# bioinformatics-ua/polus

Measured on AMD Instinct MI355X. Metric: train samples/sec BioBERT-base NER seq256, higher is better.
Workload: dtype bf16

## Files before the change

### polus_amd/csrc/attention.hip

```cpp
#include "common.h"

namespace {

constexpr int D = 64;
constexpr int BLK = 64;
constexpr float MASK_NEG = -10000.0f;
constexpr float LOG2E = 1.4426950408889634f, LN2 = 0.6931471805599453f;

template <typename T> struct TileCfg;
template <> struct TileCfg<bf16_t> { static constexpr int RS = 160, EPC = 8, LOG_CPR = 3, NLOAD = 2; };
template <> struct TileCfg<float> { static constexpr int RS = 288, EPC = 4, LOG_CPR = 4, NLOAD = 4; };

template <typename T, int NT = 256>
__device__ __forceinline__ void tile_load(unsigned char* tile, const T* __restrict__ base, long ld, int row0,
                                          int nrows, int col0, int tid) {
    constexpr int LOG = TileCfg<T>::LOG_CPR;
#pragma unroll
    for (int k = 0; k < TileCfg<T>::NLOAD; ++k) {
        int c = tid + NT * k;
        int r = c >> LOG, ch = c & ((1 << LOG) - 1);
        uint4 v = make_uint4(0, 0, 0, 0);
        if (row0 + r < nrows)
            v = *reinterpret_cast<const uint4*>(base + (long)(row0 + r) * ld + col0 + ch * TileCfg<T>::EPC);
        *reinterpret_cast<uint4*>(tile + r * TileCfg<T>::RS + ch * 16) = v;
// ... 37 lines not shown

__device__ __forceinline__ void frag_from_acc(Frag<bf16_t>& f, const f32x4& t0, const f32x4& t1) {
    f.v[0] = (bf16_t)t0[0]; f.v[1] = (bf16_t)t0[1]; f.v[2] = (bf16_t)t0[2]; f.v[3] = (bf16_t)t0[3];
    f.v[4] = (bf16_t)t1[0]; f.v[5] = (bf16_t)t1[1]; f.v[6] = (bf16_t)t1[2]; f.v[7] = (bf16_t)t1[3];
}
__device__ __forceinline__ void frag_from_acc(Frag<float>& f, const f32x4& t0, const f32x4& t1) {
    f.v[0] = t0[0]; f.v[1] = t0[1]; f.v[2] = t0[2]; f.v[3] = t0[3];
    f.v[4] = t1[0]; f.v[5] = t1[1]; f.v[6] = t1[2]; f.v[7] = t1[3];
}

__device__ __forceinline__ float col_max(float v) { v = fmaxf(v, __shfl_xor(v, 16, 64)); return fmaxf(v, __shfl_xor(v, 32, 64)); }
__device__ __forceinline__ float col_sum(float v) { v += __shfl_xor(v, 16, 64); return v + __shfl_xor(v, 32, 64); }

template <typename T>
__device__ __forceinline__ void store_acc_T(T* __restrict__ out, long ld, int row, int col0, const f32x4 (&o)[4],
                                            float mul, int g, bool valid) {
    if (!valid) return;
#pragma unroll
    for (int dt = 0; dt < 4; ++dt) {
        float v[4] = {o[dt][0] * mul, o[dt][1] * mul, o[dt][2] * mul, o[dt][3] * mul};
        store4<T>(out + (long)row * ld + col0 + dt * 16 + 4 * g, v);
    }
}

struct AttnArgs {
    const void* qkv; const int32_t* mask; void* ctx; float* lse;
    const void* dctx; const float* delta; void* dqkv;
    int B, S, A, H;
    float scale;
    unsigned drop_thresh, drop_seed;
    float drop_inv;
    const PolusDyn* dyn;
    int debug;
};

__device__ __forceinline__ float key_bias(const int32_t* mask, int b, int S, int key) {
    if (key >= S) return -INFINITY;
    if (!mask) return 0.0f;
    return (1.0f - (float)mask[(long)b * S + key]) * MASK_NEG;
}

template <typename T, int NW>
__global__ __launch_bounds__(64 * NW) void attn_fwd_kernel(AttnArgs p) {
    if (p.drop_thresh) p.drop_seed = polus_eff_seed(p.drop_seed, p.dyn);
    constexpr int QB = 16 * NW, NT = 64 * NW;
    extern __shared__ __attribute__((aligned(16))) unsigned char smem[];
    unsigned char* Kc = smem;
    unsigned char* Vc = smem + QB * TileCfg<T>::RS;
    float* kbc = reinterpret_cast<float*>(smem + 2 * QB * TileCfg<T>::RS);
    const int tid = threadIdx.x, lane = tid & 63, wid = tid >> 6, i = lane & 15, g = lane >> 4;
    const int q0 = blockIdx.x * QB, h = blockIdx.y, b = blockIdx.z;
    const int S = p.S, H = p.H;
    const long ld = 3L * H;
    const T* qkv = static_cast<const T*>(p.qkv) + (long)b * S * ld;
    const int q = q0 + wid * 16 + i;
    const bool qvalid = q < S;

    Frag<T> qf[2];
#pragma unroll
    for (int sub = 0; sub < 2; ++sub)
        frag_global<T>(qf[sub], qkv + (long)q * ld + h * D + sub * 32 + 8 * g, qvalid);

    const float scale2 = p.scale * LOG2E;
    float m = -1e30f, l = 0.f;
    f32x4 o[4];
#pragma unroll
    for (int dt = 0; dt < 4; ++dt) o[dt] = (f32x4){0.f, 0.f, 0.f, 0.f};
// ... 117 lines not shown

    auto issue_block = [&](int j) {
        unsigned char* st = ring + (j & 3) * FWD_STAGE;
#pragma unroll
        for (int e = 0; e < PPW; ++e) {
            const int piece = wid + e * NW;
            const int row = min(j * BLK + (piece & 7) * 8 + r8, S - 1);
            dma16(qkv + (long)row * ld + (piece < 8 ? H : 2 * H) + h * D + src_chunk, st + piece * 1024);
        }
    };
    const int nblk = (S + BLK - 1) / BLK;
    if (p.mask)
        for (int k0 = wid * 64; k0 < S; k0 += 64 * NW)
            dma4(p.mask + (long)b * S + min(k0 + lane, S - 1), reinterpret_cast<unsigned char*>(kbc) + k0 * 4);
    {
        unsigned char* qs = ring + 3 * FWD_STAGE;
#pragma unroll
        for (int e = 0; e < 2; ++e) {
            const int piece = wid + e * NW;
            dma16(qkv + (long)min(q0 + piece * 8 + r8, S - 1) * ld + h * D + src_chunk, qs + piece * 1024);
        }
    }
#pragma unroll
    for (int j = 0; j < 3; ++j) if (j < nblk) issue_block(j);
    wait_blocks_left<PPW>(min(nblk, 3));
    __builtin_amdgcn_s_barrier();
    Frag<T> qf[2];
    {
        const int row = wid * 16 + i;
#pragma unroll
        for (int sub = 0; sub < 2; ++sub)
            qf[sub].v = *reinterpret_cast<const bf16x8*>(ring + 3 * FWD_STAGE + row * 128 + (((sub * 4 + g) ^ (row & 7)) * 16));
    }
    for (int t = tid; t < nblk * BLK; t += NT) {
        float bias = 0.0f;
        if (p.mask) bias = (1.0f - (float)reinterpret_cast<const int*>(kbc)[t]) * MASK_NEG;
        kbc[t] = t < S ? bias * LOG2E : -INFINITY;
    }
    wait_lgkm();
    __builtin_amdgcn_s_barrier();
    if (nblk > 3) issue_block(3);
    int issued = min(nblk, 4);

    const float scale2 = p.scale * LOG2E;
    float m = -1e30f, l = 0.f;
    f32x4 o[4];
#pragma unroll
    for (int dt = 0; dt < 4; ++dt) o[dt] = (f32x4){0.f, 0.f, 0.f, 0.f};
    const int kx = i & 7;
    const int k_off0 = i * 128 + ((g ^ kx) * 16), k_off1 = i * 128 + (((4 + g) ^ kx) * 16);
    const int vrow = 4 * g + (i >> 2), vx = vrow & 7;
    const int v_base = vrow * 128 + (i & 1) * 8, v_c = (i & 3) >> 1;

    for (int j0 = 0; j0 < nblk; j0 += 2) {
        const bool two = j0 + 1 < nblk;
        f32x4 s[2][4];
#pragma unroll
        for (int jj = 0; jj < 2; ++jj) {
            if (jj == 0 || two) {
                wait_blocks_left<PPW>(issued - 1 - (j0 + jj));
                __builtin_amdgcn_s_barrier();
                const unsigned char* Kt = ring + ((j0 + jj) & 3) * FWD_STAGE;
#pragma unroll
                for (int kt = 0; kt < 4; ++kt) {
                    s[jj][kt] = (f32x4){0.f, 0.f, 0.f, 0.f};
                    Frag<T> a0, a1;
                    a0.v = *reinterpret_cast<const bf16x8*>(Kt + kt * 2048 + k_off0);
                    a1.v = *reinterpret_cast<const bf16x8*>(Kt + kt * 2048 + k_off1);
                    mma16(s[jj][kt], a0, qf[0]);
                    mma16(s[jj][kt], a1, qf[1]);
                }
            } else {
#pragma unroll
                for (int kt = 0; kt < 4; ++kt) s[jj][kt] = (f32x4){-INFINITY, -INFINITY, -INFINITY, -INFINITY};
            }
        }
        float mx = -INFINITY;
#pragma unroll
        for (int jj = 0; jj < 2; ++jj)
            if (jj == 0 || two) {
#pragma unroll
                for (int kt = 0; kt < 4; ++kt) {
                    const f32x4 kb = *reinterpret_cast<const f32x4*>(kbc + (j0 + jj) * BLK + kt * 16 + 4 * g);
#pragma unroll
                    for (int r = 0; r < 4; ++r) s[jj][kt][r] = fmaf(s[jj][kt][r], scale2, kb[r]);
                    mx = fmaxf(mx, fmaxf(fmaxf(s[jj][kt][0], s[jj][kt][1]), fmaxf(s[jj][kt][2], s[jj][kt][3])));
                }
            }
        mx = col_max2(mx);
        const float m_new = fmaxf(m, mx);
        const float alpha = __builtin_amdgcn_exp2f(m - m_new);
        m = m_new;
        float rs = 0.f;
        Frag<T> pf[2][2];
#pragma unroll
        for (int jj = 0; jj < 2; ++jj) {
#pragma unroll
            for (int kt = 0; kt < 4; ++kt)
#pragma unroll
                for (int r = 0; r < 4; ++r) { s[jj][kt][r] = __builtin_amdgcn_exp2f(s[jj][kt][r] - m_new); rs += s[jj][kt][r]; }
            if (p.drop_thresh) {
                const unsigned rowb = (((unsigned)b * p.A + h) * S + (unsigned)q) * S + (j0 + jj) * BLK + 4 * g;
#pragma unroll
                for (int kt = 0; kt < 4; ++kt) {
                    float t4[4] = {s[jj][kt][0], s[jj][kt][1], s[jj][kt][2], s[jj][kt][3]};
                    polus_dropout_run<4>(t4, p.drop_seed, rowb + kt * 16, p.drop_thresh, p.drop_inv, (S & 3) == 0);
                    s[jj][kt] = (f32x4){t4[0], t4[1], t4[2], t4[3]};
                }
            }
            frag_from_acc(pf[jj][0], s[jj][0], s[jj][1]);
            frag_from_acc(pf[jj][1], s[jj][2], s[jj][3]);
        }
        l = l * alpha + rs;
#pragma unroll
        for (int dt = 0; dt < 4; ++dt)
#pragma unroll
            for (int r = 0; r < 4; ++r) o[dt][r] *= alpha;
#pragma unroll
        for (int jj = 0; jj < 2; ++jj) {
            if (jj == 0 || two) {
                const unsigned char* Vt = ring + ((j0 + jj) & 3) * FWD_STAGE + BLK * 128 + v_base;
#pragma unroll
                for (int ks = 0; ks < 2; ++ks)
#pragma unroll
                    for (int dt = 0; dt < 4; ++dt) {
                        const unsigned char* vp = Vt + ks * 4096 + (((2 * dt + v_c) ^ vx) * 16);
                        const s16x4 lo = lds_tr16(vp), hi = lds_tr16(vp + 16 * 128);
                        typedef short s16x8 __attribute__((ext_vector_type(8)));
                        const s16x8 w = {lo[0], lo[1], lo[2], lo[3], hi[0], hi[1], hi[2], hi[3]};
                        Frag<T> va;
                        va.v = __builtin_bit_cast(bf16x8, w);
                        mma16(o[dt], va, pf[jj][ks]);
                    }
            }
        }
        if (j0 + 4 < nblk) {
            wait_lgkm();
            __builtin_amdgcn_s_barrier();
            issue_block(j0 + 4);
            ++issued;
            if (j0 + 5 < nblk) { issue_block(j0 + 5); ++issued; }
        }
    }
    l = col_sum2(l);
    const float inv_l = 1.0f / l;
    wait_lgkm();
    __builtin_amdgcn_s_barrier();
    unsigned char* ot = ring + wid * 2048;
#pragma unroll
    for (int dt = 0; dt < 4; ++dt) {
        float v[4] = {o[dt][0] * inv_l, o[dt][1] * inv_l, o[dt][2] * inv_l, o[dt][3] * inv_l};
        store4<T>(reinterpret_cast<T*>(ot + i * 128 + (((2 * dt + (g >> 1)) ^ (i & 7)) * 16) + (g & 1) * 8), v);
    }
    wait_lgkm();
    T* ctx = static_cast<T*>(p.ctx) + (long)b * S * H;
#pragma unroll
    for (int t = 0; t < 2; ++t) {
        const int row = 8 * t + r8, qq = q0 + wid * 16 + row;
        const uint4 v = *reinterpret_cast<const uint4*>(ot + row * 128 + (lane & 7) * 16);
        if (qq < S) *reinterpret_cast<uint4*>(ctx + (long)qq * H + h * D + (((lane & 7) ^ (row & 7)) * 8)) = v;
    }
    if (q < S && g == 0) p.lse[((long)b * p.A + h) * S + q] = m * LN2 + __logf(l);
}

template <typename T, int NW>
__global__ __launch_bounds__(64 * NW) void attn_bwd_dq_kernel(AttnArgs p) {
    if (p.drop_thresh) p.drop_seed = polus_eff_seed(p.drop_seed, p.dyn);
    constexpr int QB = 16 * NW, NT = 64 * NW;
// ... 343 lines not shown
__device__ __forceinline__ unsigned lds_off(const unsigned char* p) { return (unsigned)(unsigned long)(const lds_u8*)p; }
template <int ROW16>
__device__ __forceinline__ void tr_pair_asm(Frag<bf16_t>& f, unsigned addr) {
    v2i_t lo, hi;
    asm volatile("ds_read_b64_tr_b16 %0, %2\n\tds_read_b64_tr_b16 %1, %2 offset:%3" : "=&v"(lo), "=&v"(hi) : "v"(addr), "n"(ROW16));
    typedef int v4i_t __attribute__((ext_vector_type(4)));
    const v4i_t w = {lo[0], lo[1], hi[0], hi[1]};
    f.v = __builtin_bit_cast(bf16x8, w);
}
__device__ __forceinline__ void ds_read128_asm(Frag<bf16_t>& f, unsigned addr) {
    typedef int v4i_t __attribute__((ext_vector_type(4)));
    v4i_t w;
    asm volatile("ds_read_b128 %0, %1" : "=&v"(w) : "v"(addr));
    f.v = __builtin_bit_cast(bf16x8, w);
}
__device__ __forceinline__ uint2 ds_read64_asm(unsigned addr) {
    v2i_t w;
    asm volatile("ds_read_b64 %0, %1" : "=&v"(w) : "v"(addr));
    return make_uint2((unsigned)w[0], (unsigned)w[1]);
}
__device__ __forceinline__ void lds_fence() {
    asm volatile("s_waitcnt lgkmcnt(0)" ::: "memory");
    __builtin_amdgcn_sched_barrier(0);
}
template <int R> __device__ __forceinline__ unsigned quad_bcast(unsigned v) {
    return (unsigned)__builtin_amdgcn_mov_dpp((int)v, R | (R << 2) | (R << 4) | (R << 6), 0xF, 0xF, true);
}


constexpr int Q64_KB = 64;
template <int NW> struct Q64Cfg {
    static constexpr int S = 16 * NW;
    static constexpr int OFF_O = S * 128, OFF_K = 2 * S * 128, OFF_V = OFF_K + Q64_KB * 128, OFF_P = OFF_V + Q64_KB * 128,
                         OFF_D = OFF_P + 4 * S * 32, OFF_B = OFF_D + 4 * S * 32, SMEM = OFF_B + S * 4;
};

template <int NW>
__global__ __launch_bounds__(64 * NW, 4) void attn_bwd_q64_kernel(AttnArgs p) {
    typedef bf16_t T;
    typedef Q64Cfg<NW> C;
    constexpr int S = C::S, NT = 64 * NW, NKB = S / Q64_KB;
    constexpr int KVP = 16 / NW;
    constexpr int COMBOS = NW >= 8 ? 1 : 8 / NW;
    constexpr int KTW = NW == 16 ? 2 : 4;
    if (p.drop_thresh) p.drop_seed = polus_eff_seed(p.drop_seed, p.dyn);
    extern __shared__ __attribute__((aligned(16))) unsigned char smem[];
    unsigned char* Qi = smem;
    unsigned char* Oi = smem + C::OFF_O;
    unsigned char* Kb = smem + C::OFF_K;
    unsigned char* Vb = smem + C::OFF_V;
    unsigned char* Ps = smem + C::OFF_P;
    unsigned char* Ds = smem + C::OFF_D;
    float* kbc = reinterpret_cast<float*>(smem + C::OFF_B);
    const int tid = threadIdx.x, lane = tid & 63, i = lane & 15, g = lane >> 4;
    const int wid = __builtin_amdgcn_readfirstlane(tid >> 6);
    const int h = blockIdx.x, b = blockIdx.y;
    const int H = p.H;
    const long ld = 3L * H;
    const T* qkv = static_cast<const T*>(p.qkv) + (long)b * S * ld;
    const T* dctx = static_cast<const T*>(p.dctx) + (long)b * S * H;
    T* dqkv = static_cast<T*>(p.dqkv) + (long)b * S * ld;
    const int q = wid * 16 + i;
    const int r8 = lane >> 3, src_chunk = ((lane & 7) ^ r8) * 8;

    auto issue_kv = [&](int kb) {
#pragma unroll
        for (int e = 0; e < KVP; ++e) {
            const int piece = wid + e * NW;
            const long row = (long)(kb * Q64_KB + (piece & 7) * 8 + r8) * ld + h * D + src_chunk;
            dma16(qkv + row + (piece < 8 ? H : 2 * H), (piece < 8 ? Kb : Vb) + (piece & 7) * 1024);
        }
    };
#pragma unroll
    for (int e = 0; e < 2; ++e) {
        const int piece = wid + e * NW;
        dma16(qkv + (long)(piece * 8 + r8) * ld + h * D + src_chunk, Qi + piece * 1024);
        dma16(dctx + (long)(piece * 8 + r8) * H + h * D + src_chunk, Oi + piece * 1024);
    }
    issue_kv(0);
    if (tid < S) kbc[tid] = key_bias(p.mask, b, S, tid) * LOG2E;
    const long stat = ((long)b * p.A + h) * S + q;
    const float lse2 = p.lse[stat] * LOG2E;
    const float scale2 = p.scale * LOG2E;
    Frag<T> of[2];
    {
        const T* ctx = static_cast<const T*>(p.ctx) + (long)b * S * H;
#pragma unroll
        for (int sub = 0; sub < 2; ++sub) frag_global<T>(of[sub], ctx + (long)q * H + h * D + sub * 32 + 8 * g, true);
    }
    wait_vm<0>();
    wait_lgkm();
    __builtin_amdgcn_s_barrier();
    const int qoff0 = q * 128 + ((g ^ (q & 7)) * 16), qoff1 = q * 128 + (((4 + g) ^ (q & 7)) * 16);
    float dl = 0.f;
    {
        Frag<T> dof[2];
        ds_read128_asm(dof[0], lds_off(Oi + qoff0));
        ds_read128_asm(dof[1], lds_off(Oi + qoff1));
        lds_fence();
#pragma unroll
        for (int sub = 0; sub < 2; ++sub)
#pragma unroll
            for (int j = 0; j < 8; ++j) dl += (float)of[sub].v[j] * (float)dof[sub].v[j];
        dl = col_sum(dl);
    }
    f32x4 dq[4];
#pragma unroll
    for (int dt = 0; dt < 4; ++dt) dq[dt] = (f32x4){0.f, 0.f, 0.f, 0.f};

    const int rr0 = i * 128 + ((g ^ (i & 7)) * 16), rr1 = i * 128 + (((4 + g) ^ (i & 7)) * 16);
    const int trow = 4 * g + (i >> 2), tx = trow & 7, thalf = (i & 1) * 8, tc = (i & 3) >> 1;
    const int st_w = q * 32 + ((g ^ ((q >> 2) & 3)) * 8);
    const int st_r = trow * 32 + (((i & 3) ^ g) * 8);

    for (int kb = 0; kb < NKB; ++kb) {
        f32x4 s[4];
        Frag<T> qf[2], dof[2];
        ds_read128_asm(qf[0], lds_off(Qi + qoff0));
        ds_read128_asm(qf[1], lds_off(Qi + qoff1));
        ds_read128_asm(dof[0], lds_off(Oi + qoff0));
        ds_read128_asm(dof[1], lds_off(Oi + qoff1));
        const unsigned rowb = (((unsigned)b * p.A + h) * S + (unsigned)q) * S + kb * Q64_KB + 4 * g;
#pragma unroll
        for (int kt = 0; kt < 4; ++kt) {
            Frag<T> ka[2], va[2];
            ds_read128_asm(ka[0], lds_off(Kb + kt * 2048 + rr0));
            ds_read128_asm(ka[1], lds_off(Kb + kt * 2048 + rr1));
            ds_read128_asm(va[0], lds_off(Vb + kt * 2048 + rr0));
            ds_read128_asm(va[1], lds_off(Vb + kt * 2048 + rr1));
            lds_fence();
            f32x4 dp = (f32x4){0.f, 0.f, 0.f, 0.f};
            s[kt] = (f32x4){0.f, 0.f, 0.f, 0.f};
            mma16(s[kt], ka[0], qf[0]);
            mma16(s[kt], ka[1], qf[1]);
            mma16(dp, va[0], dof[0]);
            mma16(dp, va[1], dof[1]);
            float pd[4], dsv[4];
            bool keep[4] = {true, true, true, true};
            if (p.drop_thresh) polus_keep4(p.drop_seed, rowb + kt * 16, p.drop_thresh, keep);
            const f32x4 kbv = *reinterpret_cast<const f32x4*>(kbc + kb * Q64_KB + kt * 16 + 4 * g);
#pragma unroll
            for (int r = 0; r < 4; ++r) {
                const float pr = __builtin_amdgcn_exp2f(fmaf(s[kt][r], scale2, kbv[r]) - lse2);
                const float pk = keep[r] ? pr * p.drop_inv : 0.f;
                const float dpe = keep[r] ? dp[r] * p.drop_inv : 0.f;
                pd[r] = pk;
                dsv[r] = pr * (dpe - dl) * p.scale;
                s[kt][r] = dsv[r];
            }
            store4<T>(reinterpret_cast<T*>(Ps + kt * (S * 32) + st_w), pd);
            store4<T>(reinterpret_cast<T*>(Ds + kt * (S * 32) + st_w), dsv);
        }
        {
            Frag<T> kT[2][4];
#pragma unroll
            for (int ks = 0; ks < 2; ++ks)
#pragma unroll
                for (int dt = 0; dt < 4; ++dt)
                    tr_pair_asm<16 * 128>(kT[ks][dt], lds_off(Kb + (ks * 32 + trow) * 128 + (((2 * dt + tc) ^ tx) * 16) + thalf));
            lds_fence();
#pragma unroll
            for (int ks = 0; ks < 2; ++ks) {
                Frag<T> dsb;
                frag_from_acc(dsb, s[2 * ks], s[2 * ks + 1]);
#pragma unroll
                for (int dt = 0; dt < 4; ++dt) mma16(dq[dt], kT[ks][dt], dsb);
            }
        }
        wait_lgkm();
        __builtin_amdgcn_s_barrier();
        if (kb + 1 < NKB) issue_kv(kb + 1);
#pragma unroll
        for (int c = 0; c < COMBOS; ++c) {
            const int combo = NW == 16 ? (wid >> 1) : wid * COMBOS + c;
            const int type = combo >> 2, dt = combo & 3, kt0 = NW == 16 ? (wid & 1) * 2 : 0;
            const unsigned char* At = type ? Oi : Qi;
            const unsigned char* Bt = type ? Ps : Ds;
            constexpr int QH = (S / 32) < 4 ? (S / 32) : 4;
            f32x4 acc[KTW];
#pragma unroll
            for (int k2 = 0; k2 < KTW; ++k2) acc[k2] = (f32x4){0.f, 0.f, 0.f, 0.f};
#pragma unroll
            for (int q0 = 0; q0 < S / 32; q0 += QH) {
                Frag<T> af[QH];
#pragma unroll
                for (int qs = 0; qs < QH; ++qs)
                    tr_pair_asm<16 * 128>(af[qs], lds_off(At + ((q0 + qs) * 32 + trow) * 128 + (((2 * dt + tc) ^ tx) * 16) + thalf));
#pragma unroll
                for (int k2 = 0; k2 < KTW; ++k2) {
                    Frag<T> bf[QH];
#pragma unroll
                    for (int qs = 0; qs < QH; ++qs)
                        tr_pair_asm<16 * 32>(bf[qs], lds_off(Bt + (kt0 + k2) * (S * 32) + (q0 + qs) * 32 * 32 + st_r));
                    lds_fence();
#pragma unroll
                    for (int qs = 0; qs < QH; ++qs) mma16(acc[k2], af[qs], bf[qs]);
                }
            }
#pragma unroll
            for (int k2 = 0; k2 < KTW; ++k2) {
                float v[4] = {acc[k2][0], acc[k2][1], acc[k2][2], acc[k2][3]};
                store4<T>(dqkv + (long)(kb * Q64_KB + (kt0 + k2) * 16 + i) * ld + (type ? 2 * H : H) + h * D + dt * 16 + 4 * g, v);
            }
        }
        if (kb + 1 < NKB) wait_vm<COMBOS * KTW>();
        wait_lgkm();
        __builtin_amdgcn_s_barrier();
    }
    store_acc_T<T>(dqkv, ld, q, h * D, dq, 1.0f, g, true);
}

constexpr int KR_KEYS = 256, KR_QS = 32, KR_RING = 4;
constexpr int KR_KV = KR_KEYS * 128;
constexpr int KR_SLICE = KR_QS * 128;
// ... 254 lines not shown
}

__global__ __launch_bounds__(256) void attn_bwd_dq_finish_kernel(const float* __restrict__ slabs, bf16_t* __restrict__ dqkv,
                                                                  long rows, int H, int nkb) {
    const long n4 = rows * (H / 4);
    for (long e = (long)blockIdx.x * blockDim.x + threadIdx.x; e < n4; e += (long)gridDim.x * blockDim.x) {
        const long row = e / (H / 4);
        const int c = (int)(e - row * (H / 4)) * 4;
        float4 a = *reinterpret_cast<const float4*>(slabs + row * H + c);
        for (int k = 1; k < nkb; ++k) {
            const float4 v = *reinterpret_cast<const float4*>(slabs + ((long)k * rows + row) * H + c);
            a.x += v.x; a.y += v.y; a.z += v.z; a.w += v.w;
        }
        float v[4] = {a.x, a.y, a.z, a.w};
        store4<bf16_t>(dqkv + row * 3L * H + c, v);
    }
}

int check_common(const char* who, int dtype, int B, int S, int A, int hd) {
    POLUS_REQUIRE(dtype == POLUS_F32 || dtype == POLUS_BF16, "%s: bad dtype %d", who, dtype);
    POLUS_REQUIRE(hd == D, "%s: head_dim must be 64 (got %d)", who, hd);
    POLUS_REQUIRE(B > 0 && S > 0 && A > 0, "%s: bad shape B=%d S=%d A=%d", who, B, S, A);
    POLUS_REQUIRE(B <= 65535 && A <= 65535, "%s: B and n_heads must be <= 65535", who);
    return POLUS_OK;
}

}

namespace {
template <int WHICH, typename T, int NW>
int launch_wide_nw(const AttnArgs& a, hipStream_t st) {
    auto kern = WHICH == 0 ? attn_fwd_kernel<T, NW> : attn_bwd_dq_kernel<T, NW>;
    constexpr int QB = 16 * NW;
    const size_t lds = 2 * (size_t)QB * TileCfg<T>::RS + QB * 4;
    static bool attr_done = false;
    if (!attr_done && lds > 48 * 1024) {
        POLUS_HIP(hipFuncSetAttribute(reinterpret_cast<const void*>(kern), hipFuncAttributeMaxDynamicSharedMemorySize, (int)lds));
        attr_done = true;
    }
    dim3 grid((a.S + QB - 1) / QB, a.A, a.B);
    hipLaunchKernelGGL(kern, grid, dim3(64 * NW), lds, st, a);
    return POLUS_OK;
}
template <int NW>
int launch_fwd_dma(const AttnArgs& a, hipStream_t st) {
    auto kern = attn_fwd_dma_kernel<NW>;
    const size_t lds = FWD_RING * FWD_STAGE + (size_t)((a.S + 64 * NW - 1) / (64 * NW)) * 64 * NW * 4;
    static bool attr_done = false;
    if (!attr_done) {
        POLUS_HIP(hipFuncSetAttribute(reinterpret_cast<const void*>(kern), hipFuncAttributeMaxDynamicSharedMemorySize,
                                      FWD_RING * FWD_STAGE + (FWD_MAX_S + 64 * NW) * 4));
        attr_done = true;
    }
    hipLaunchKernelGGL(kern, dim3((a.S + 16 * NW - 1) / (16 * NW), a.A, a.B), dim3(64 * NW), lds, st, a);
    return POLUS_OK;
}
template <int NW>
int launch_q64(const AttnArgs& a, int n_heads, int B, hipStream_t st) {
    auto kern = attn_bwd_q64_kernel<NW>;
    static bool attr_done = false;
    if (!attr_done) {
        POLUS_HIP(hipFuncSetAttribute(reinterpret_cast<const void*>(kern), hipFuncAttributeMaxDynamicSharedMemorySize, Q64Cfg<NW>::SMEM));
        attr_done = true;
    }
    hipLaunchKernelGGL(kern, dim3(n_heads, B), dim3(64 * NW), Q64Cfg<NW>::SMEM, st, a);
    return POLUS_OK;
}
template <int NW>
int launch_fused(const AttnArgs& a, int n_heads, int B, size_t lds, hipStream_t st) {
    auto kern = attn_bwd_fused_kernel<NW>;
    static bool attr_done = false;
    if (!attr_done) {
        POLUS_HIP(hipFuncSetAttribute(reinterpret_cast<const void*>(kern), hipFuncAttributeMaxDynamicSharedMemorySize, (int)lds));
        attr_done = true;
    }
    hipLaunchKernelGGL(kern, dim3(n_heads, B), dim3(64 * NW), lds, st, a);
    return POLUS_OK;
}
template <int WHICH>
int launch_wide(int dtype, const AttnArgs& a, hipStream_t st) {
    if (dtype != POLUS_BF16) return launch_wide_nw<WHICH, float, 4>(a, st);
    if (a.S >= 96) return launch_wide_nw<WHICH, bf16_t, 8>(a, st);
    return launch_wide_nw<WHICH, bf16_t, 4>(a, st);
}
}

extern "C" int polus_attention_fwd(int dtype, const void* qkv, const int32_t* mask, void* ctx, float* lse,
                                   int B, int S, int n_heads, int head_dim, float drop_p, uint32_t seed, void* stream) {
    int rc = check_common("polus_attention_fwd", dtype, B, S, n_heads, head_dim);
    if (rc) return rc;
    POLUS_REQUIRE(qkv && ctx && lse, "polus_attention_fwd: null pointer");
    POLUS_REQUIRE(polus_aligned16(qkv) && polus_aligned16(ctx), "polus_attention_fwd: pointers must be 16-byte aligned");
    AttnArgs a = {};
    POLUS_REQUIRE(drop_p >= 0.f && drop_p < 1.f && (long)B * n_heads * S * S < (1LL << 32), "polus_attention_fwd: bad dropout arguments");
    a.qkv = qkv; a.mask = mask; a.ctx = ctx; a.lse = lse;
    a.B = B; a.S = S; a.A = n_heads; a.H = n_heads * D; a.scale = 0.125f;
    a.drop_thresh = drop_p > 0.f ? polus_drop_thresh(drop_p) : 0u; a.drop_seed = seed; a.drop_inv = 1.0f / (1.0f - drop_p); a.dyn = polus_dyn();
    hipStream_t st = static_cast<hipStream_t>(stream);
    int rc2;
    if (dtype == POLUS_BF16 && S <= FWD_MAX_S)
        rc2 = S >= 96 ? launch_fwd_dma<8>(a, st) : launch_fwd_dma<4>(a, st);
    else
        rc2 = launch_wide<0>(dtype, a, st);
    if (rc2 != POLUS_OK) return rc2;
    POLUS_CHECK_LAUNCH("polus_attention_fwd");
    return POLUS_OK;
}

extern "C" size_t polus_attention_bwd_workspace_bytes(int B, int S, int n_heads) {
    size_t n = (size_t)B * S * n_heads * sizeof(float);
    if (S > KR_KEYS && S % KR_KEYS == 0 && S <= 2048) n += (size_t)(S / KR_KEYS) * B * S * n_heads * D * sizeof(float);
    return n;
}

extern "C" int polus_attention_bwd(int dtype, const void* qkv, const int32_t* mask, const void* ctx,
                                   const void* dctx, const float* lse, void* dqkv,
                                   int B, int S, int n_heads, int head_dim, float drop_p, uint32_t seed,
                                   void* workspace, size_t workspace_bytes, void* stream) {
    int rc = check_common("polus_attention_bwd", dtype, B, S, n_heads, head_dim);
    if (rc) return rc;
    POLUS_REQUIRE(qkv && ctx && dctx && lse && dqkv, "polus_attention_bwd: null pointer");
    POLUS_REQUIRE(polus_aligned16(qkv) && polus_aligned16(ctx) && polus_aligned16(dctx) && polus_aligned16(dqkv),
                  "polus_attention_bwd: pointers must be 16-byte aligned");
    size_t need = polus_attention_bwd_workspace_bytes(B, S, n_heads);
    if (!workspace || workspace_bytes < need) { polus_set_error("polus_attention_bwd: workspace %zu < %zu", workspace_bytes, need); return POLUS_ERR_WORKSPACE; }
    AttnArgs a = {};
    a.qkv = qkv; a.mask = mask; a.ctx = const_cast<void*>(ctx); a.lse = const_cast<float*>(lse); a.dctx = dctx; a.dqkv = dqkv;
    a.delta = static_cast<const float*>(workspace);
    a.B = B; a.S = S; a.A = n_heads; a.H = n_heads * D; a.scale = 0.125f;
    POLUS_REQUIRE(drop_p >= 0.f && drop_p < 1.f && (long)B * n_heads * S * S < (1LL << 32), "polus_attention_bwd: bad dropout arguments");
    a.drop_thresh = drop_p > 0.f ? polus_drop_thresh(drop_p) : 0u; a.drop_seed = seed; a.drop_inv = 1.0f / (1.0f - drop_p); a.dyn = polus_dyn();
    a.debug = polus_cfg().attn_debug;
    hipStream_t st = static_cast<hipStream_t>(stream);
    dim3 grid((S + BLK - 1) / BLK, n_heads, B);
    const int kres = polus_cfg().attn_bwd_kres;
    if (dtype == POLUS_BF16 && polus_cfg().attn_fused && kres && S % KR_KEYS == 0 && S <= 2048 && (S > KR_KEYS || kres >= 2)) {
        const int nkb = S / KR_KEYS;
        float* slabs = nkb > 1 ? static_cast<float*>(workspace) + (size_t)B * S * n_heads : nullptr;
        const size_t lds = KR_OFF_STAT + 2 * (size_t)S * sizeof(float);
        static bool attr_done = false;
        if (!attr_done) {
            POLUS_HIP(hipFuncSetAttribute(reinterpret_cast<const void*>(attn_bwd_kres_kernel), hipFuncAttributeMaxDynamicSharedMemorySize, 160 * 1024));
            attr_done = true;
        }
        hipLaunchKernelGGL(attn_bwd_kres_kernel, dim3(nkb, n_heads, B), dim3(512), lds, st, a, slabs);
        POLUS_CHECK_LAUNCH("polus_attention_bwd(key-resident)");
        if (nkb > 1) {
            hipLaunchKernelGGL(attn_bwd_dq_finish_kernel, dim3(1024), dim3(256), 0, st, slabs, static_cast<bf16_t*>(dqkv), (long)B * S, a.H, nkb);
            POLUS_CHECK_LAUNCH("polus_attention_bwd(dQ slabs)");
        }
        return POLUS_OK;
    }
    const int fused = polus_cfg().attn_fused;
    if (dtype == POLUS_BF16 && fused && S == 256) {
        int rc2 = launch_q64<16>(a, n_heads, B, st);
        if (rc2 != POLUS_OK) return rc2;
        POLUS_CHECK_LAUNCH("polus_attention_bwd(one pass, 64-key blocks)");
        return POLUS_OK;
    }
    if (dtype == POLUS_BF16 && fused && (S == 64 || S == 128)) {
        const size_t lds = 2 * (size_t)S * TileCfg<bf16_t>::RS + 4 * (size_t)KBLK * TileCfg<bf16_t>::RS + 2 * (size_t)S * RSS + (size_t)S * 4;
        int rc2 = S == 128 ? launch_fused<8>(a, n_heads, B, lds, st) : launch_fused<4>(a, n_heads, B, lds, st);
        if (rc2 != POLUS_OK) return rc2;
        POLUS_CHECK_LAUNCH("polus_attention_bwd(fused)");
        return POLUS_OK;
    }
    if (dtype == POLUS_BF16) {
        { int rc2 = launch_wide<1>(dtype, a, st); if (rc2 != POLUS_OK) return rc2; }
        POLUS_CHECK_LAUNCH("polus_attention_bwd(dq)");
        hipLaunchKernelGGL(attn_bwd_dkv_kernel<bf16_t>, grid, dim3(256), 0, st, a);
    } else {
        { int rc2 = launch_wide<1>(dtype, a, st); if (rc2 != POLUS_OK) return rc2; }
        POLUS_CHECK_LAUNCH("polus_attention_bwd(dq)");
        hipLaunchKernelGGL(attn_bwd_dkv_kernel<float>, grid, dim3(256), 0, st, a);
    }
    POLUS_CHECK_LAUNCH("polus_attention_bwd(dkv)");
    return POLUS_OK;
}
```

### polus_amd/csrc/common.h

```cpp
#pragma once
#include <hip/hip_runtime.h>
#include <stdint.h>
#include <stdio.h>
#include <string.h>
#include <math.h>

#include "../../include/polus_hip.h"

typedef __bf16 bf16_t;
typedef __bf16 bf16x8 __attribute__((ext_vector_type(8)));
typedef __bf16 bf16x4 __attribute__((ext_vector_type(4)));
typedef short s16x4 __attribute__((ext_vector_type(4)));
typedef float f32x4 __attribute__((ext_vector_type(4)));

void polus_set_error(const char* fmt, ...);
#define POLUS_FAIL(...) do { polus_set_error(__VA_ARGS__); return POLUS_ERR_INVALID; } while (0)
#define POLUS_REQUIRE(cond, ...) do { if (!(cond)) { polus_set_error(__VA_ARGS__); return POLUS_ERR_INVALID; } } while (0)
#define POLUS_CHECK_LAUNCH(name) do { hipError_t e__ = hipGetLastError(); \
    if (e__ != hipSuccess) { polus_set_error("%s: launch failed: %s", name, hipGetErrorString(e__)); return POLUS_ERR_HIP; } } while (0)
#define POLUS_HIP(call) do { hipError_t e__ = (call); \
    if (e__ != hipSuccess) { polus_set_error("%s failed: %s", #call, hipGetErrorString(e__)); return POLUS_ERR_HIP; } } while (0)

static inline size_t polus_dtype_size(int dt) { return dt == POLUS_BF16 ? 2 : 4; }
static inline bool polus_aligned16(const void* p) { return (((uintptr_t)p) & 15) == 0; }

struct PolusCfg {
    int gemm_pp;
    int gemm_v1;
    int dw_ungrouped;
    int dw_fused_reduce;
    int ln_bwd_blocks;
    int ln_fin_single;
    int gemm_ring128;
    int gemm_auto_split;
    int ln_halfwave;
    int gemm_order;
    int gemm_persist;
    int reserve_cus;
    int attn_bwd_kres;
    int attn_debug;
    int dw_streamk;
    int dw_sk_cus;
    int dw_sk_delta;
    int attn_fused;
};
const PolusCfg& polus_cfg();
int polus_num_cus();
int polus_reserved_cus();

struct PolusDyn { uint32_t salt; float lr, lr_t; uint32_t pad; };
const PolusDyn* polus_dyn();
__device__ __forceinline__ uint32_t polus_eff_seed(uint32_t seed, const PolusDyn* dyn) {
    if (!dyn) return seed;
    uint32_t x = seed + dyn->salt;
    x ^= x >> 15;
    return x * 0x2C1B3C6Du;
}

template <typename T> __device__ __forceinline__ float to_f(T x);
template <> __device__ __forceinline__ float to_f<float>(float x) { return x; }
template <> __device__ __forceinline__ float to_f<bf16_t>(bf16_t x) { return (float)x; }
template <typename T> __device__ __forceinline__ T from_f(float x);
template <> __device__ __forceinline__ float from_f<float>(float x) { return x; }
template <> __device__ __forceinline__ bf16_t from_f<bf16_t>(float x) { return (bf16_t)x; }

template <typename T> __device__ __forceinline__ void load4(const T* p, float (&v)[4]);
template <> __device__ __forceinline__ void load4<float>(const float* p, float (&v)[4]) {
    float4 t = *reinterpret_cast<const float4*>(p); v[0] = t.x; v[1] = t.y; v[2] = t.z; v[3] = t.w;
}
template <> __device__ __forceinline__ void load4<bf16_t>(const bf16_t* p, float (&v)[4]) {
    bf16x4 t = *reinterpret_cast<const bf16x4*>(p);
    v[0] = (float)t[0]; v[1] = (float)t[1]; v[2] = (float)t[2]; v[3] = (float)t[3];
}
template <typename T> __device__ __forceinline__ void store4(T* p, const float (&v)[4]);
template <> __device__ __forceinline__ void store4<float>(float* p, const float (&v)[4]) {
    *reinterpret_cast<float4*>(p) = make_float4(v[0], v[1], v[2], v[3]);
// ... 65 lines not shown
        for (int r = 0; r < N; ++r) v[r] = swish_f(v[r]);
    } else if (act == POLUS_ACT_RELU) {
#pragma unroll
        for (int r = 0; r < N; ++r) v[r] = fmaxf(v[r], 0.0f);
    } else if (act == POLUS_ACT_TANH) {
#pragma unroll
        for (int r = 0; r < N; ++r) v[r] = tanhf(v[r]);
    }
}
template <int N, bool FAST = false> __device__ __forceinline__ void apply_act_grad_n(int act, float (&v)[N], const float (&u)[N]) {
    if (act == POLUS_ACT_GELU) {
        if (FAST && (N % 2) == 0) {
#pragma unroll
            for (int r = 0; r < N; r += 2) {
                f32x2_t d = (f32x2_t){v[r], v[r + 1]} * gelu_grad2((f32x2_t){u[r], u[r + 1]});
                v[r] = d[0]; v[r + 1] = d[1];
            }
            return;
        }
#pragma unroll
        for (int r = 0; r < N; ++r) v[r] *= gelu_grad_f(u[r]);
    } else if (act == POLUS_ACT_SWISH) {
#pragma unroll
        for (int r = 0; r < N; ++r) v[r] *= swish_grad_f(u[r]);
    } else if (act == POLUS_ACT_RELU) {
#pragma unroll
        for (int r = 0; r < N; ++r) v[r] = u[r] > 0.0f ? v[r] : 0.0f;
    } else if (act == POLUS_ACT_TANH) {
#pragma unroll
        for (int r = 0; r < N; ++r) { float t = tanhf(u[r]); v[r] *= 1.0f - t * t; }
    }
}

__device__ __forceinline__ uint32_t polus_hash32(uint32_t seed, uint32_t idx) {
    uint32_t x = idx * 0x9E3779B1u + seed;
    x ^= x >> 16; x *= 0x85EBCA6Bu;
    x ^= x >> 13; x *= 0xC2B2AE35u;
    x ^= x >> 16;
    return x;
}
__device__ __forceinline__ uint32_t polus_hash32_second(uint32_t h1) {
    uint32_t y = h1 * 0x27D4EB2Fu;
    return y ^ (y >> 15);
}
__device__ __forceinline__ bool polus_keep(uint32_t seed, uint32_t idx, uint32_t thresh) {
    const uint32_t h1 = polus_hash32(seed, idx >> 2);
    const uint32_t h = (idx & 2u) ? polus_hash32_second(h1) : h1;
    return ((idx & 1u) ? (h >> 16) : (h & 0xFFFFu)) >= thresh;
}
__device__ __forceinline__ void polus_keep4(uint32_t seed, uint32_t idx4, uint32_t thresh, bool (&k)[4]) {
    const uint32_t h1 = polus_hash32(seed, idx4 >> 2), h2 = polus_hash32_second(h1);
    k[0] = (h1 & 0xFFFFu) >= thresh;
    k[1] = (h1 >> 16) >= thresh;
    k[2] = (h2 & 0xFFFFu) >= thresh;
    k[3] = (h2 >> 16) >= thresh;
}
template <int N>
__device__ __forceinline__ void polus_dropout_run(float (&v)[N], uint32_t seed, uint32_t base, uint32_t thresh, float inv, bool quad) {
    static_assert(N % 4 == 0, "runs of whole quads");
    if (quad) {
#pragma unroll
        for (int r = 0; r < N; r += 4) {
            bool k[4];
            polus_keep4(seed, base + r, thresh, k);
#pragma unroll
            for (int e = 0; e < 4; ++e) v[r + e] = k[e] ? v[r + e] * inv : 0.f;
        }
    } else {
#pragma unroll
        for (int r = 0; r < N; ++r) v[r] = polus_keep(seed, base + r, thresh) ? v[r] * inv : 0.f;
    }
}
static inline uint32_t polus_drop_thresh(float p) {
    double t = (double)p * 65536.0 + 0.5;
    return t <= 0.0 ? 0u : (t >= 65535.0 ? 65535u : (uint32_t)t);
}

__device__ __forceinline__ float wave_sum(float v) {
#pragma unroll
    for (int o = 32; o > 0; o >>= 1) v += __shfl_xor(v, o, 64);
    return v;
}
__device__ __forceinline__ float wave_max(float v) {
#pragma unroll
    for (int o = 32; o > 0; o >>= 1) v = fmaxf(v, __shfl_xor(v, o, 64));
    return v;
}

// ... 28 lines not shown
```

### polus_amd/csrc/runtime.hip

```cpp
#include "common.h"
#include <stdarg.h>

static thread_local char g_err[512] = "";

void polus_set_error(const char* fmt, ...) {
    va_list ap;
    va_start(ap, fmt);
    vsnprintf(g_err, sizeof(g_err), fmt, ap);
    va_end(ap);
}

extern "C" const char* polus_last_error(void) { return g_err; }

static PolusCfg g_cfg;
static bool g_cfg_ready = false;
static int env_int(const char* name, int dflt) {
    const char* e = getenv(name);
    return (e && *e) ? atoi(e) : dflt;
}
static void read_cfg() {
    g_cfg.gemm_pp = env_int("POLUS_GEMM_PP", 0);
    g_cfg.gemm_v1 = getenv("POLUS_GEMM_V1") != nullptr;
    g_cfg.dw_ungrouped = getenv("POLUS_DW_UNGROUPED") != nullptr;
    g_cfg.gemm_order = env_int("POLUS_GEMM_ORDER", 4);
    g_cfg.reserve_cus = env_int("POLUS_GEMM_RESERVE_CUS", 0);
    g_cfg.gemm_persist = env_int("POLUS_GEMM_PERSIST", 1);
    g_cfg.dw_fused_reduce = env_int("POLUS_DW_FUSED_REDUCE", 1);
    g_cfg.attn_fused = env_int("POLUS_ATTN_FUSED", 1);
    g_cfg.attn_bwd_kres = env_int("POLUS_ATTN_BWD_KRES", 1);
    g_cfg.attn_debug = env_int("POLUS_ATTN_DEBUG", 0);
    g_cfg.ln_halfwave = env_int("POLUS_LN_HALFWAVE", 1);
    g_cfg.gemm_auto_split = env_int("POLUS_GEMM_AUTO_SPLIT", 1);
    g_cfg.gemm_ring128 = env_int("POLUS_GEMM_RING128", 0);
    g_cfg.ln_bwd_blocks = env_int("POLUS_LN_BWD_BLOCKS", 512);
    g_cfg.ln_fin_single = env_int("POLUS_LN_FIN_SINGLE", 512);
    g_cfg.dw_streamk = env_int("POLUS_DW_STREAMK", 0);
    g_cfg.dw_sk_delta = env_int("POLUS_DW_SK_DELTA", 2);
    g_cfg.dw_sk_cus = env_int("POLUS_DW_SK_CUS", 0);
    g_cfg_ready = true;
}
const PolusCfg& polus_cfg() {
    if (!g_cfg_ready) read_cfg();
    return g_cfg;
}
extern "C" int polus_reload_env(void) { read_cfg(); return POLUS_OK; }

int polus_num_cus() {
    static int n = 0;
    if (!n) {
        int dev = 0; hipDeviceProp_t prop;
        if (hipGetDevice(&dev) == hipSuccess && hipGetDeviceProperties(&prop, dev) == hipSuccess) n = prop.multiProcessorCount;
        if (n <= 0) n = 256;
    }
    return n;
}
static int g_reserve_on = 1;
extern "C" int polus_set_reserve_active(int on) { g_reserve_on = on != 0; return POLUS_OK; }
int polus_reserved_cus() { return g_reserve_on ? polus_cfg().reserve_cus : 0; }

static const PolusDyn* g_dyn = nullptr;
const PolusDyn* polus_dyn() { return g_dyn; }
extern "C" int polus_set_dynamic_params(const void* dev_block16) {
    POLUS_REQUIRE(dev_block16 == nullptr || polus_aligned16(dev_block16), "polus_set_dynamic_params: the block must be 16-byte aligned");
// ... 246 lines not shown
```

Baseline: 5388.

## Skip fully padded key blocks in attention forward and backward kernels

While building the key-bias table, each block now records a per-64-key-block flag saying whether any key in that block is unmasked, using a wave ballot. In both the forward DMA kernel and the backward dQ kernel, key blocks that are entirely padding skip their QK, softmax, dropout and PV/dS matrix work. The loads and barriers still run so the pipeline stays in step. The dropout hash base is also precomputed once per row, and dS is written straight to bf16 instead of going through float staging. The cost is a small extra LDS region and a new env toggle, POLUS_ATTN_SKIP, on by default; the gain depends on how much padding the batches carry.

```diff
diff --git a/polus_amd/csrc/attention.hip b/polus_amd/csrc/attention.hip
--- a/polus_amd/csrc/attention.hip
+++ b/polus_amd/csrc/attention.hip
@@ -93,7 +93,9 @@
     float drop_inv;
     const PolusDyn* dyn;
     int debug;
+    int skip;
 };
+
 
 __device__ __forceinline__ float key_bias(const int32_t* mask, int b, int S, int key) {
     if (key >= S) return -INFINITY;
@@ -277,13 +279,24 @@
         for (int sub = 0; sub < 2; ++sub)
             qf[sub].v = *reinterpret_cast<const bf16x8*>(ring + 3 * FWD_STAGE + row * 128 + (((sub * 4 + g) ^ (row & 7)) * 16));
     }
+    int* bflag = reinterpret_cast<int*>(kbc + (S + 64 * NW - 1) / (64 * NW) * (64 * NW));
     for (int t = tid; t < nblk * BLK; t += NT) {
         float bias = 0.0f;
-        if (p.mask) bias = (1.0f - (float)reinterpret_cast<const int*>(kbc)[t]) * MASK_NEG;
+        int mv = 1;
+        if (p.mask) { mv = reinterpret_cast<const int*>(kbc)[t]; bias = (1.0f - (float)mv) * MASK_NEG; }
         kbc[t] = t < S ? bias * LOG2E : -INFINITY;
+        const unsigned long long any = __ballot(t < S && mv > 0);
+        if (lane == 0) bflag[t >> 6] = any != 0ull;
     }
     wait_lgkm();
     __builtin_amdgcn_s_barrier();
+    unsigned live = ~0u;
+    if (p.skip && p.mask) {
+        unsigned l = 0;
+        for (int j = 0; j < nblk; ++j) l |= (bflag[j] ? 1u : 0u) << j;
+        l = __builtin_amdgcn_readfirstlane(l);
+        if (l) live = l;
+    }
     if (nblk > 3) issue_block(3);
     int issued = min(nblk, 4);
 
@@ -297,14 +310,19 @@
     const int vrow = 4 * g + (i >> 2), vx = vrow & 7;
     const int v_base = vrow * 128 + (i & 1) * 8, v_c = (i & 3) >> 1;
 
+    const bool quad = (S & 3) == 0;
+    const uint32_t x0 = ((((unsigned)b * p.A + h) * S + (unsigned)q) * S + 4 * g) / 4 * POLUS_HASH_MUL + p.drop_seed;
     for (int j0 = 0; j0 < nblk; j0 += 2) {
         const bool two = j0 + 1 < nblk;
+        const bool use[2] = {((live >> j0) & 1u) != 0, two && ((live >> (j0 + 1)) & 1u) != 0};
         f32x4 s[2][4];
 #pragma unroll
         for (int jj = 0; jj < 2; ++jj) {
             if (jj == 0 || two) {
                 wait_blocks_left<PPW>(issued - 1 - (j0 + jj));
                 __builtin_amdgcn_s_barrier();
+            }
+            if (use[jj]) {
                 const unsigned char* Kt = ring + ((j0 + jj) & 3) * FWD_STAGE;
 #pragma unroll
                 for (int kt = 0; kt < 4; ++kt) {
@@ -315,15 +333,13 @@
                     mma16(s[jj][kt], a0, qf[0]);
                     mma16(s[jj][kt], a1, qf[1]);
                 }
-            } else {
-#pragma unroll
-                for (int kt = 0; kt < 4; ++kt) s[jj][kt] = (f32x4){-INFINITY, -INFINITY, -INFINITY, -INFINITY};
-            }
-        }
+            }
+        }
+      if (use[0] || use[1]) {
         float mx = -INFINITY;
 #pragma unroll
         for (int jj = 0; jj < 2; ++jj)
-            if (jj == 0 || two) {
+            if (use[jj]) {
 #pragma unroll
                 for (int kt = 0; kt < 4; ++kt) {
                     const f32x4 kb = *reinterpret_cast<const f32x4*>(kbc + (j0 + jj) * BLK + kt * 16 + 4 * g);
@@ -340,6 +356,7 @@
         Frag<T> pf[2][2];
 #pragma unroll
         for (int jj = 0; jj < 2; ++jj) {
+            if (!use[jj]) continue;
 #pragma unroll
             for (int kt = 0; kt < 4; ++kt)
 #pragma unroll
@@ -348,9 +365,14 @@
                 const unsigned rowb = (((unsigned)b * p.A + h) * S + (unsigned)q) * S + (j0 + jj) * BLK + 4 * g;
 #pragma unroll
                 for (int kt = 0; kt < 4; ++kt) {
-                    float t4[4] = {s[jj][kt][0], s[jj][kt][1], s[jj][kt][2], s[jj][kt][3]};
-                    polus_dropout_run<4>(t4, p.drop_seed, rowb + kt * 16, p.drop_thresh, p.drop_inv, (S & 3) == 0);
-                    s[jj][kt] = (f32x4){t4[0], t4[1], t4[2], t4[3]};
+                    bool k[4];
+                    if (quad) polus_keep4_x(x0 + (unsigned)(16 * (j0 + jj) + 4 * kt) * POLUS_HASH_MUL, p.drop_thresh, k);
+                    else {
+#pragma unroll
+                        for (int r = 0; r < 4; ++r) k[r] = polus_keep(p.drop_seed, rowb + kt * 16 + r, p.drop_thresh);
+                    }
+#pragma unroll
+                    for (int r = 0; r < 4; ++r) s[jj][kt][r] = k[r] ? s[jj][kt][r] * p.drop_inv : 0.f;
                 }
             }
             frag_from_acc(pf[jj][0], s[jj][0], s[jj][1]);
@@ -363,7 +385,7 @@
             for (int r = 0; r < 4; ++r) o[dt][r] *= alpha;
 #pragma unroll
         for (int jj = 0; jj < 2; ++jj) {
-            if (jj == 0 || two) {
+            if (use[jj]) {
                 const unsigned char* Vt = ring + ((j0 + jj) & 3) * FWD_STAGE + BLK * 128 + v_base;
 #pragma unroll
                 for (int ks = 0; ks < 2; ++ks)
@@ -379,6 +401,7 @@
                     }
             }
         }
+      }
         if (j0 + 4 < nblk) {
             wait_lgkm();
             __builtin_amdgcn_s_barrier();
@@ -788,7 +811,7 @@
 template <int NW> struct Q64Cfg {
     static constexpr int S = 16 * NW;
     static constexpr int OFF_O = S * 128, OFF_K = 2 * S * 128, OFF_V = OFF_K + Q64_KB * 128, OFF_P = OFF_V + Q64_KB * 128,
-                         OFF_D = OFF_P + 4 * S * 32, OFF_B = OFF_D + 4 * S * 32, SMEM = OFF_B + S * 4;
+                         OFF_D = OFF_P + 4 * S * 32, OFF_B = OFF_D + 4 * S * 32, OFF_F = OFF_B + S * 4, SMEM = OFF_F + 16;
 };
 
 template <int NW>
@@ -799,6 +822,7 @@
     constexpr int KVP = 16 / NW;
     constexpr int COMBOS = NW >= 8 ? 1 : 8 / NW;
     constexpr int KTW = NW == 16 ? 2 : 4;
+    static_assert(NKB <= 32, "one flag bit per key block");
     if (p.drop_thresh) p.drop_seed = polus_eff_seed(p.drop_seed, p.dyn);
     extern __shared__ __attribute__((aligned(16))) unsigned char smem[];
     unsigned char* Qi = smem;
@@ -808,6 +832,7 @@
     unsigned char* Ps = smem + C::OFF_P;
     unsigned char* Ds = smem + C::OFF_D;
     float* kbc = reinterpret_cast<float*>(smem + C::OFF_B);
+    int* bflag = reinterpret_cast<int*>(smem + C::OFF_F);
     const int tid = threadIdx.x, lane = tid & 63, i = lane & 15, g = lane >> 4;
     const int wid = __builtin_amdgcn_readfirstlane(tid >> 6);
     const int h = blockIdx.x, b = blockIdx.y;
@@ -834,7 +859,12 @@
         dma16(dctx + (long)(piece * 8 + r8) * H + h * D + src_chunk, Oi + piece * 1024);
     }
     issue_kv(0);
-    if (tid < S) kbc[tid] = key_bias(p.mask, b, S, tid) * LOG2E;
+    if (tid < S) {
+        const int mv = p.mask ? p.mask[(long)b * S + tid] : 1;
+        kbc[tid] = (p.mask ? (1.0f - (float)mv) * MASK_NEG : 0.0f) * LOG2E;
+        const unsigned long long any = __ballot(mv > 0);
+        if (lane == 0) bflag[wid] = any != 0ull;
+    }
     const long stat = ((long)b * p.A + h) * S + q;
     const float lse2 = p.lse[stat] * LOG2E;
     const float scale2 = p.scale * LOG2E;
@@ -847,6 +877,14 @@
     wait_vm<0>();
     wait_lgkm();
     __builtin_amdgcn_s_barrier();
+    unsigned live = (1u << NKB) - 1;
+    if (p.skip && p.mask) {
+        unsigned l = 0;
+#pragma unroll
+        for (int j = 0; j < NKB; ++j) l |= (bflag[j] ? 1u : 0u) << j;
+        l = __builtin_amdgcn_readfirstlane(l);
+        if (l) live = l;
+    }
     const int qoff0 = q * 128 + ((g ^ (q & 7)) * 16), qoff1 = q * 128 + (((4 + g) ^ (q & 7)) * 16);
     float dl = 0.f;
     {
@@ -869,14 +907,17 @@
     const int st_w = q * 32 + ((g ^ ((q >> 2) & 3)) * 8);
     const int st_r = trow * 32 + (((i & 3) ^ g) * 8);
 
+    const uint32_t x0 = ((((unsigned)b * p.A + h) * S + (unsigned)q) * (S / 4) + g) * POLUS_HASH_MUL + p.drop_seed;
     for (int kb = 0; kb < NKB; ++kb) {
+        const bool use = (live >> kb) & 1u;
+      if (use) {
         f32x4 s[4];
+        bf16x4 ds16[4];
         Frag<T> qf[2], dof[2];
         ds_read128_asm(qf[0], lds_off(Qi + qoff0));
         ds_read128_asm(qf[1], lds_off(Qi + qoff1));
         ds_read128_asm(dof[0], lds_off(Oi + qoff0));
         ds_read128_asm(dof[1], lds_off(Oi + qoff1));
-        const unsigned rowb = (((unsigned)b * p.A + h) * S + (unsigned)q) * S + kb * Q64_KB + 4 * g;
 #pragma unroll
         for (int kt = 0; kt < 4; ++kt) {
             Frag<T> ka[2], va[2];
@@ -891,9 +932,9 @@
             mma16(s[kt], ka[1], qf[1]);
             mma16(dp, va[0], dof[0]);
             mma16(dp, va[1], dof[1]);
-            float pd[4], dsv[4];
+            float pd[4];
             bool keep[4] = {true, true, true, true};
-            if (p.drop_thresh) polus_keep4(p.drop_seed, rowb + kt * 16, p.drop_thresh, keep);
+            if (p.drop_thresh) polus_keep4_x(x0 + (unsigned)(16 * kb + 4 * kt) * POLUS_HASH_MUL, p.drop_thresh, keep);
             const f32x4 kbv = *reinterpret_cast<const f32x4*>(kbc + kb * Q64_KB + kt * 16 + 4 * g);
 #pragma unroll
             for (int r = 0; r < 4; ++r) {
@@ -901,11 +942,10 @@
                 const float pk = keep[r] ? pr * p.drop_inv : 0.f;
                 const float dpe = keep[r] ? dp[r] * p.drop_inv : 0.f;
                 pd[r] = pk;
-                dsv[r] = pr * (dpe - dl) * p.scale;
-                s[kt][r] = dsv[r];
+                ds16[kt][r] = (bf16_t)(pr * (dpe - dl) * p.scale);
             }
             store4<T>(reinterpret_cast<T*>(Ps + kt * (S * 32) + st_w), pd);
-            store4<T>(reinterpret_cast<T*>(Ds + kt * (S * 32) + st_w), dsv);
+            *reinterpret_cast<bf16x4*>(Ds + kt * (S * 32) + st_w) = ds16[kt];
         }
         {
             Frag<T> kT[2][4];
@@ -918,11 +958,12 @@
 #pragma unroll
             for (int ks = 0; ks < 2; ++ks) {
                 Frag<T> dsb;
-                frag_from_acc(dsb, s[2 * ks], s[2 * ks + 1]);
+                dsb.v = __builtin_shufflevector(ds16[2 * ks], ds16[2 * ks + 1], 0, 1, 2, 3, 4, 5, 6, 7);
 #pragma unroll
                 for (int dt = 0; dt < 4; ++dt) mma16(dq[dt], kT[ks][dt], dsb);
             }
         }
+      }
         wait_lgkm();
         __builtin_amdgcn_s_barrier();
         if (kb + 1 < NKB) issue_kv(kb + 1);
@@ -936,6 +977,7 @@
             f32x4 acc[KTW];
 #pragma unroll
             for (int k2 = 0; k2 < KTW; ++k2) acc[k2] = (f32x4){0.f, 0.f, 0.f, 0.f};
+            if (use)
 #pragma unroll
             for (int q0 = 0; q0 < S / 32; q0 += QH) {
                 Frag<T> af[QH];
@@ -1256,9 +1298,9 @@
 int launch_wide_nw(const AttnArgs& a, hipStream_t st) {
     auto kern = WHICH == 0 ? attn_fwd_kernel<T, NW> : attn_bwd_dq_kernel<T, NW>;
     constexpr int QB = 16 * NW;
-    const size_t lds = 2 * (size_t)QB * TileCfg<T>::RS + QB * 4;
+    constexpr size_t lds = 2 * (size_t)QB * TileCfg<T>::RS + QB * 4;
     static bool attr_done = false;
-    if (!attr_done && lds > 48 * 1024) {
+    if (!attr_done) {
         POLUS_HIP(hipFuncSetAttribute(reinterpret_cast<const void*>(kern), hipFuncAttributeMaxDynamicSharedMemorySize, (int)lds));
         attr_done = true;
     }
@@ -1269,11 +1311,11 @@
 template <int NW>
 int launch_fwd_dma(const AttnArgs& a, hipStream_t st) {
     auto kern = attn_fwd_dma_kernel<NW>;
-    const size_t lds = FWD_RING * FWD_STAGE + (size_t)((a.S + 64 * NW - 1) / (64 * NW)) * 64 * NW * 4;
+    const size_t lds = FWD_RING * FWD_STAGE + (size_t)((a.S + 64 * NW - 1) / (64 * NW)) * 64 * NW * 4 + 64;
     static bool attr_done = false;
     if (!attr_done) {
         POLUS_HIP(hipFuncSetAttribute(reinterpret_cast<const void*>(kern), hipFuncAttributeMaxDynamicSharedMemorySize,
-                                      FWD_RING * FWD_STAGE + (FWD_MAX_S + 64 * NW) * 4));
+                                      FWD_RING * FWD_STAGE + (FWD_MAX_S + 64 * NW) * 4 + 64));
         attr_done = true;
     }
     hipLaunchKernelGGL(kern, dim3((a.S + 16 * NW - 1) / (16 * NW), a.A, a.B), dim3(64 * NW), lds, st, a);
@@ -1291,8 +1333,10 @@
     return POLUS_OK;
 }
 template <int NW>
-int launch_fused(const AttnArgs& a, int n_heads, int B, size_t lds, hipStream_t st) {
+int launch_fused(const AttnArgs& a, int n_heads, int B, hipStream_t st) {
     auto kern = attn_bwd_fused_kernel<NW>;
+    constexpr int S = 16 * NW;
+    constexpr size_t lds = 2 * (size_t)S * TileCfg<bf16_t>::RS + 4 * (size_t)KBLK * TileCfg<bf16_t>::RS + 2 * (size_t)S * RSS + (size_t)S * 4;
     static bool attr_done = false;
     if (!attr_done) {
         POLUS_HIP(hipFuncSetAttribute(reinterpret_cast<const void*>(kern), hipFuncAttributeMaxDynamicSharedMemorySize, (int)lds));
@@ -1320,6 +1364,7 @@
     a.qkv = qkv; a.mask = mask; a.ctx = ctx; a.lse = lse;
     a.B = B; a.S = S; a.A = n_heads; a.H = n_heads * D; a.scale = 0.125f;
     a.drop_thresh = drop_p > 0.f ? polus_drop_thresh(drop_p) : 0u; a.drop_seed = seed; a.drop_inv = 1.0f / (1.0f - drop_p); a.dyn = polus_dyn();
+    a.skip = polus_cfg().attn_skip;
     hipStream_t st = static_cast<hipStream_t>(stream);
     int rc2;
     if (dtype == POLUS_BF16 && S <= FWD_MAX_S)
@@ -1355,6 +1400,7 @@
     POLUS_REQUIRE(drop_p >= 0.f && drop_p < 1.f && (long)B * n_heads * S * S < (1LL << 32), "polus_attention_bwd: bad dropout arguments");
     a.drop_thresh = drop_p > 0.f ? polus_drop_thresh(drop_p) : 0u; a.drop_seed = seed; a.drop_inv = 1.0f / (1.0f - drop_p); a.dyn = polus_dyn();
     a.debug = polus_cfg().attn_debug;
+    a.skip = polus_cfg().attn_skip;
     hipStream_t st = static_cast<hipStream_t>(stream);
     dim3 grid((S + BLK - 1) / BLK, n_heads, B);
     const int kres = polus_cfg().attn_bwd_kres;
@@ -1383,8 +1429,7 @@
         return POLUS_OK;
     }
     if (dtype == POLUS_BF16 && fused && (S == 64 || S == 128)) {
-        const size_t lds = 2 * (size_t)S * TileCfg<bf16_t>::RS + 4 * (size_t)KBLK * TileCfg<bf16_t>::RS + 2 * (size_t)S * RSS + (size_t)S * 4;
-        int rc2 = S == 128 ? launch_fused<8>(a, n_heads, B, lds, st) : launch_fused<4>(a, n_heads, B, lds, st);
+        int rc2 = S == 128 ? launch_fused<8>(a, n_heads, B, st) : launch_fused<4>(a, n_heads, B, st);
         if (rc2 != POLUS_OK) return rc2;
         POLUS_CHECK_LAUNCH("polus_attention_bwd(fused)");
         return POLUS_OK;
diff --git a/polus_amd/csrc/common.h b/polus_amd/csrc/common.h
--- a/polus_amd/csrc/common.h
+++ b/polus_amd/csrc/common.h
@@ -42,6 +42,7 @@
     int dw_streamk;
     int dw_sk_cus;
     int dw_sk_delta;
+    int attn_skip;
     int attn_fused;
 };
 const PolusCfg& polus_cfg();
@@ -173,13 +174,14 @@
     }
 }
 
-__device__ __forceinline__ uint32_t polus_hash32(uint32_t seed, uint32_t idx) {
-    uint32_t x = idx * 0x9E3779B1u + seed;
+constexpr uint32_t POLUS_HASH_MUL = 0x9E3779B1u;
+__device__ __forceinline__ uint32_t polus_hash32_x(uint32_t x) {
     x ^= x >> 16; x *= 0x85EBCA6Bu;
     x ^= x >> 13; x *= 0xC2B2AE35u;
     x ^= x >> 16;
     return x;
 }
+__device__ __forceinline__ uint32_t polus_hash32(uint32_t seed, uint32_t idx) { return polus_hash32_x(idx * POLUS_HASH_MUL + seed); }
 __device__ __forceinline__ uint32_t polus_hash32_second(uint32_t h1) {
     uint32_t y = h1 * 0x27D4EB2Fu;
     return y ^ (y >> 15);
@@ -189,12 +191,15 @@
     const uint32_t h = (idx & 2u) ? polus_hash32_second(h1) : h1;
     return ((idx & 1u) ? (h >> 16) : (h & 0xFFFFu)) >= thresh;
 }
-__device__ __forceinline__ void polus_keep4(uint32_t seed, uint32_t idx4, uint32_t thresh, bool (&k)[4]) {
-    const uint32_t h1 = polus_hash32(seed, idx4 >> 2), h2 = polus_hash32_second(h1);
+__device__ __forceinline__ void polus_keep4_x(uint32_t x, uint32_t thresh, bool (&k)[4]) {
+    const uint32_t h1 = polus_hash32_x(x), h2 = polus_hash32_second(h1);
     k[0] = (h1 & 0xFFFFu) >= thresh;
     k[1] = (h1 >> 16) >= thresh;
     k[2] = (h2 & 0xFFFFu) >= thresh;
     k[3] = (h2 >> 16) >= thresh;
+}
+__device__ __forceinline__ void polus_keep4(uint32_t seed, uint32_t idx4, uint32_t thresh, bool (&k)[4]) {
+    polus_keep4_x((idx4 >> 2) * POLUS_HASH_MUL + seed, thresh, k);
 }
 template <int N>
 __device__ __forceinline__ void polus_dropout_run(float (&v)[N], uint32_t seed, uint32_t base, uint32_t thresh, float inv, bool quad) {
diff --git a/polus_amd/csrc/runtime.hip b/polus_amd/csrc/runtime.hip
--- a/polus_amd/csrc/runtime.hip
+++ b/polus_amd/csrc/runtime.hip
@@ -29,6 +29,7 @@
     g_cfg.attn_fused = env_int("POLUS_ATTN_FUSED", 1);
     g_cfg.attn_bwd_kres = env_int("POLUS_ATTN_BWD_KRES", 1);
     g_cfg.attn_debug = env_int("POLUS_ATTN_DEBUG", 0);
+    g_cfg.attn_skip = env_int("POLUS_ATTN_SKIP", 1);
     g_cfg.ln_halfwave = env_int("POLUS_LN_HALFWAVE", 1);
     g_cfg.gemm_auto_split = env_int("POLUS_GEMM_AUTO_SPLIT", 1);
     g_cfg.gemm_ring128 = env_int("POLUS_GEMM_RING128", 0);
```

Result: no change. 5430 (median of 6 runs) (+0.8%).
